# RmSchaffert/ACCV-Lab

Hardware: AMD Instinct MI355X
Metric: heatmap frames/sec (1920x1080 fp32, ragged N_obj in [1,128], fused clear+draw) (higher is better)
Workload: dtype f32

## Files before the change

accv-lab_amd/accvlab/_amd_native/__init__.py:

```python
from __future__ import annotations

import ctypes
import os

_HERE = os.path.dirname(os.path.abspath(__file__))
NO_HOST_FASTPATH = os.environ.get("ACCV_NO_HOST_FASTPATH", "") not in ("", "0")
LIB_PATH = os.environ.get("ACCV_HIP_LIB") or os.path.join(_HERE, "libaccv_hip.so")

OK = 0
HM_CLEAR = 1
HM_COUNTS_I64 = 2
HM_SMALL_RADII = 4
HM_WRITE_THROUGH = 8
HM_GROUP_BOXES_GIVEN = 16
HM_TILE_ROWS_16 = 32
HM_TILE_ROWS_8 = 64
HM_CALLER_SCALE_ORDER = 256
HM_PLAIN_STORES = 128
HM_POINT_COUNTS_I64 = 512
MP_IDX_I64 = 1
MP_COUNTS_I64 = 2
MP_LABELS_I64 = 4
FL_AVG_NUM_POS = 0
FL_AVG_VALUE = 1
FL_AVG_DEVICE = 2
LSA_MAXIMIZE = 1
LSA_THREADS_64 = 2
LSA_THREADS_1024 = 4
MC_ONE_MINUS_PROB = 0
MC_NEG_PROB = 1
MC_FOCAL = 2
MC_LABELS_I64 = 1
MC_CXCYWH = 2
CR_MAX_MAPS = 8
CR_MAX_CHANNELS = 64
CR_COUNTS_I64 = 1
CR_INDEX_FORM = 2
CR_WEIGHTS_PER_CHANNEL = 4
CR_L1 = 0
CR_SMOOTH_L1 = 2
MF_IDX_I64 = 1
MF_LABELS_I64 = 2
MB_IDX_I64 = 1
MB_CXCYWH = 2
MB_IOU_NONE = 0
MB_IOU = 1
MB_GIOU = 2
MB_MAX_D = 16
PM_IDX_I64 = 1
PM_REVERSIBLE = 2
PM_LABELS_I64 = 4
PM_CLOSED_I32 = 8
PM_CLOSED_I64 = 16
PM_MIN_P = 2
PM_MAX_P = 128
CT_MAX_TASKS = 8
CT_MAX_CLASSES = 64
CT_NO_TASK = 255
CT_LABELS_I64 = 1
CT_COUNTS_I64 = 2
CD_MAX_TASKS = 8
CD_MAX_MAPS = 8
CD_MAX_CLASSES = 64
CD_MAX_K = 1024
RN_MAX_TASKS = 8
RN_MAX_N = 1024
RN_MIN_D = 7
RN_MAX_D = 16

_vp = ctypes.c_void_p
_i = ctypes.c_int
_f = ctypes.c_float
_u = ctypes.c_uint
_sz = ctypes.c_size_t
_i64 = ctypes.c_int64
_ll = ctypes.c_longlong
_u64 = ctypes.c_uint64

SIGNATURES = {
    "accv_last_error": (ctypes.c_char_p, []),
    "accv_version": (_i, []),
    "accv_draw_heatmap_last_dispatch": (ctypes.c_char_p, []),
    "accv_draw_heatmap_time_next_launch": (_i, [_vp, _vp]),
    "accv_draw_heatmap_flat_workspace_bytes": (_sz, [_i, _i]),
    "accv_draw_heatmap_flat_f32": (_i, [_vp, _i, _i, _i, _vp, _vp, _vp, _i, _f, _f, _u, _vp, _sz, _vp]),
    "accv_draw_heatmap_batched_f32": (_i, [_vp, _i, _i, _i, _i, _vp, _vp, _vp, _vp, _i, _f, _f, _u, _vp]),
    "accv_fill_f32": (_i, [_vp, _sz, _f, _vp]),
    "accv_draw_heatmap_multiscale_f32": (_i, [_vp, _vp, _vp, _vp, _i, _i, _vp, _vp, _vp, _i, _f, _f, _u, _vp]),
    "accv_draw_heatmap_multiscale_sample_f32": (_i, [_vp, _vp, _vp, _vp, _i, _i, _vp, _vp, _vp, _i, _f, _f, _u,
                                                      _vp, _i, _i, _vp, _i, _vp, _vp, _vp]),
    "accv_draw_points_workspace_bytes": (_sz, [_i, _i]),
    "accv_draw_points_multiscale_f32": (_i, [_vp, _vp, _vp, _vp, _i, _i, _vp, _vp, _i, _i, _f, _f, _u, _vp, _sz, _vp]),
    "accv_draw_polylines_fused_applicable": (_i, [_vp, _vp, _i, _i, _i, _i, _i]),
    "accv_draw_polylines_multiscale_f32": (_i, [_vp, _vp, _vp, _vp, _i, _i, _vp, _i, _i, _vp, _vp, _i, _i, _f, _f, _u, _vp]),
    "accv_heatmap_targets_from_boxes_f32": (_i, [_vp, _vp, _ll, _f, _vp, _vp, _vp]),
    "accv_heatmap_targets_from_points_f32": (_i, [_vp, _ll, _f, _i, _vp, _vp, _vp]),
    "accv_ragged_gather": (_i, [_vp, _vp, _vp, _vp, _ll, _ll, _ll, _ll, _ll, _i, _i, _vp, _vp]),
    "accv_ragged_gather_fill": (_i, [_vp, _vp, _vp, _vp, _ll, _ll, _ll, _ll, _ll, _u64, _i, _i, _i, _vp, _vp]),
    "accv_ragged_scatter": (_i, [_vp, _vp, _vp, _vp, _ll, _ll, _ll, _ll, _ll, _i, _i, _vp, _vp]),
    "accv_ragged_map_pairs": (_i, [_vp, _vp, _vp, _vp, _vp, _ll, _ll, _ll, _ll, _ll, _ll, _i, _i, _vp, _vp]),
    "accv_ragged_insert_const": (_i, [_vp, _vp, _vp, _ll, _ll, _ll, _ll, _ll, _u64, _i, _i, _i, _vp, _vp]),
    "accv_ragged_pad_fill": (_i, [_vp, _vp, _ll, _ll, _ll, _u64, _i, _i, _vp]),
# ... 290 lines not shown
```

accv-lab_amd/accvlab/draw_heatmap/ops.py:

```python
from __future__ import annotations

import ctypes
from typing import Optional

import torch

from .. import _amd_native as _nat

try:
    from . import _dh_host as _dh
except ImportError:
    _dh = None
_native_bound = False


def _native():
    global _native_bound
    if _dh is None or _nat.NO_HOST_FASTPATH:
        return None
    if not _native_bound:
        h = _nat.ctypes_lib()
        addr = lambda name: ctypes.cast(getattr(h, name), ctypes.c_void_p).value
        _dh.bind_native(addr("accv_draw_heatmap_batched_f32"), addr("accv_last_error"))
        _native_bound = True
    return _dh


_FORCED_FLAGS = 0


def _hint_flags(clear: bool, small_radii: bool, write_through: bool, tile_rows) -> int:
    if tile_rows not in (None, 8, 16):
        raise RuntimeError("tile_rows must be None, 8 or 16")
    return (_nat.HM_CLEAR if clear else 0) | (_nat.HM_SMALL_RADII if small_radii else 0) | \
        (0 if write_through is None else _nat.HM_WRITE_THROUGH if write_through else _nat.HM_PLAIN_STORES) | \
        (_nat.HM_TILE_ROWS_16 if tile_rows == 16 else _nat.HM_TILE_ROWS_8 if tile_rows == 8 else 0) | _FORCED_FLAGS


def _one_launch_maps(maps, batch: int, device):
    k = len(maps)
    if not 1 <= k <= 4:
        return None
    ptrs, hs, ws = [], [], []
    for hm in maps:
        if not (isinstance(hm, torch.Tensor) and hm.is_cuda and hm.dtype == torch.float32 and hm.is_contiguous() and
                hm.device == device):
            return None
        shape = hm.shape
        if len(shape) != 3 or shape[0] != batch:
            return None
        ptr = hm.data_ptr()
        if shape[2] % 4 or ptr % 16 or shape[1] * shape[2] * 4 >= (1 << 31):
            return None
        ptrs.append(ptr)
        hs.append(shape[1])
        ws.append(shape[2])
    return (ctypes.c_void_p * k)(*ptrs), (ctypes.c_int * k)(*hs), (ctypes.c_int * k)(*ws)


def _check_maps(maps, batch: int, device, owner: str) -> None:
    for hm in maps:
        _check_input(hm, "heatmap")
        _check_dtype(hm, torch.float32, "heatmap")
        if not (hm.dim() == 3 and hm.size(0) == batch):
            raise RuntimeError("every heatmap must be of shape [batch_size, height, width]")
        if not (hm.device == device):
            raise RuntimeError(f"every heatmap must be on the {owner}' device ({device})")


def _require(cond: bool, msg: str) -> None:
    if not cond:
        raise RuntimeError(msg)


def _check_input(t: torch.Tensor, name: str) -> None:
    if not (isinstance(t, torch.Tensor)):
        raise RuntimeError(f"{name} must be a torch.Tensor")
    if not (t.is_cuda):
        raise RuntimeError(f"{name} must be a CUDA tensor")
    if not (t.is_contiguous()):
        raise RuntimeError(f"{name} must be contiguous")


def _check_dtype(t: torch.Tensor, dtype: torch.dtype, name: str) -> None:
    if not (t.dtype == dtype):
        raise RuntimeError(f"{name}: expected scalar type {dtype} but found {t.dtype}")


def _same_device(ref: torch.Tensor, *others) -> None:
    for name, t in others:
        if not (t.device == ref.device):
            raise RuntimeError(f"{name} must be on the same device as the heatmap ({ref.device})")


_FLAT_DIRECT_MAX_OBJECTS = 2048
_FLAT_DIRECT_MAX_ROUNDS = 200_000
_constants: dict = {}


def _flat_direct(planes: int, height: int, width: int, n: int) -> bool:
    if not (0 < n <= _FLAT_DIRECT_MAX_OBJECTS and 0 < planes <= 65535 and height > 0 and width > 0):
        return False
    tiles = planes * ((width + 127) // 128) * ((height + 15) // 16)
    return tiles * ((n + 63) // 64) <= _FLAT_DIRECT_MAX_ROUNDS


def _device_constant(key, make) -> torch.Tensor:
    t = _constants.get(key)
    if t is None:
        t = make()
        if torch.cuda.is_current_stream_capturing():
            return t
        torch.cuda.current_stream(t.device).synchronize()
        if len(_constants) > 256:
            _constants.clear()
        _constants[key] = t
    return t


def draw_heatmap(
    heatmaps: torch.Tensor,
    centers: torch.Tensor,
    radii: torch.Tensor,
    heatmap_idxes: torch.Tensor,
    diameter_to_sigma_factor: float = 6.0,
    k_scale: float = 1.0,
    *,
    clear: bool = False,
    small_radii: bool = False,
    write_through: Optional[bool] = None,
    tile_rows: Optional[int] = None,
) -> None:
    _check_input(heatmaps, "heatmap")
    _check_input(centers, "centers")
    _check_input(radii, "radii")
    _check_input(heatmap_idxes, "heatmap_idxes")
    if not (centers.size(0) == radii.size(0)):
        raise RuntimeError("centers and radii must have the same size at dim0")
    if not (centers.size(0) == heatmap_idxes.size(0)):
        raise RuntimeError("centers and heatmap_idxes must have the same size at dim0")
    if not (heatmaps.dim() == 3):
        raise RuntimeError("heatmap must be of shape [num_heatmaps, height, width]")
    if not (centers.dim() == 2 and centers.size(1) == 2):
        raise RuntimeError("centers must be of shape [num_targets, 2]")
    if not (radii.dim() == 1 and heatmap_idxes.dim() == 1):
        raise RuntimeError("radii and heatmap_idxes must be of shape [num_targets]")
    _check_dtype(heatmaps, torch.float32, "heatmap")
    _check_dtype(centers, torch.int32, "centers")
    _check_dtype(radii, torch.int32, "radii")
    _check_dtype(heatmap_idxes, torch.int32, "heatmap_idxes")
    _same_device(heatmaps, ("centers", centers), ("radii", radii), ("heatmap_idxes", heatmap_idxes))

    lib = _nat.lib()
    planes, height, width = heatmaps.shape
    n = centers.size(0)
    if _flat_direct(planes, height, width, n):
        with _nat.device_guard(heatmaps.device):
            dev = heatmaps.device
            count = _device_constant(("count", n, dev), lambda: torch.full((1,), n, dtype=torch.int32, device=dev))
            status = lib.accv_draw_heatmap_batched_f32(
                heatmaps.data_ptr(), 1, planes, height, width, centers.data_ptr(), radii.data_ptr(), count.data_ptr(),
                heatmap_idxes.data_ptr(), n, float(diameter_to_sigma_factor), float(k_scale),
                _hint_flags(clear, small_radii, write_through, tile_rows), _nat.stream_ptr(heatmaps.device))
        _nat.check(status, "draw_heatmap")
        return
    with _nat.device_guard(heatmaps.device):
        ws_bytes = lib.accv_draw_heatmap_flat_workspace_bytes(planes, n)
        ws = torch.empty(ws_bytes, dtype=torch.uint8, device=heatmaps.device)
        status = lib.accv_draw_heatmap_flat_f32(
            heatmaps.data_ptr(), planes, height, width, centers.data_ptr(), radii.data_ptr(),
            heatmap_idxes.data_ptr(), n, float(diameter_to_sigma_factor), float(k_scale),
            _hint_flags(clear, small_radii, write_through, tile_rows), ws.data_ptr(), ws_bytes,
            _nat.stream_ptr(heatmaps.device))
    _nat.check(status, "draw_heatmap")


def draw_heatmap_batched(
    heatmap: torch.Tensor,
    centers,
    radii,
    diameter_to_sigma_factor: float = 6.0,
    k_scale: float = 1.0,
    labels=None,
    *,
    clear: bool = False,
    small_radii: bool = False,
    write_through: Optional[bool] = None,
    tile_rows: Optional[int] = None,
) -> None:
    centers_t = centers.tensor
    radii_t = radii.tensor
    assert centers_t.shape[0] == radii_t.shape[0], "centers and radii must have the same size batch size"
    assert centers_t.shape[1] == radii_t.shape[1], "centers and radii must have the same maximum number of objects"
    counts = centers.sample_sizes
    labels_t: Optional[torch.Tensor] = None
    if labels is not None:
        labels_t = labels.tensor
        assert centers_t.shape[0] == labels_t.shape[0], "centers and labels must have the same size batch size"
        assert centers_t.shape[1] == labels_t.shape[1], \
            "centers and labels must have the same maximum number of objects"

    native = _native()
    if native is not None and isinstance(heatmap, torch.Tensor) and isinstance(counts, torch.Tensor) and \
            native.draw_batched(heatmap, centers_t, radii_t, counts, labels_t, float(diameter_to_sigma_factor), float(k_scale),
                                _hint_flags(clear, small_radii, write_through, tile_rows)):
        return

    if counts.dtype not in (torch.int32, torch.int64):
        counts = counts.to(torch.int64)

    _check_input(heatmap, "heatmap")
    _check_input(centers_t, "centers")
    _check_input(radii_t, "radii")
    _check_input(counts, "nums_targets")
    batch = heatmap.size(0)
    n_max = radii_t.size(1) if radii_t.dim() >= 2 else -1
    _require(batch == radii_t.size(0) and batch == centers_t.size(0) and batch == counts.size(0),
             "batch_size (dim 0) need to be the same for all inputs")
    if not (centers_t.dim() == 3 and centers_t.size(2) == 2):
        raise RuntimeError("centers must be of shape [batch_size, num_targets, 2]")
    if not (radii_t.dim() == 2):
        raise RuntimeError("radii must be of shape [batch_size, num_targets]")
    if not (n_max == centers_t.size(1)):
        raise RuntimeError("maximum number of targets (dim 1) need to be the same centers and radii")
    if not (counts.dim() == 1):
        raise RuntimeError("nums_targets must be of shape [batch_size]")
    _check_dtype(heatmap, torch.float32, "heatmap")
    _check_dtype(centers_t, torch.int32, "centers")
    _check_dtype(radii_t, torch.int32, "radii")
    others = [("centers", centers_t), ("radii", radii_t), ("nums_targets", counts)]
    if labels_t is None:
        if not (heatmap.dim() == 3):
            raise RuntimeError("heatmap must be of shape [batch_size, height, width]")
        num_classes, (height, width) = 0, heatmap.shape[1:]
        labels_ptr = None
    else:
        _check_input(labels_t, "labels")
        if not (heatmap.dim() == 4):
            raise RuntimeError("heatmap must be of shape [batch_size, max_num_classes, height, width]")
        if not (labels_t.dim() == 2):
            raise RuntimeError("labels must be of shape [batch_size, radii.size(1)]")
        _require(labels_t.size(0) == batch and labels_t.size(1) == n_max,
                 "labels shape must be [batch_size, radii.size(1)]")
        _check_dtype(labels_t, torch.int32, "labels")
        num_classes, height, width = heatmap.shape[1:]
        if not (num_classes > 0 or heatmap.numel() == 0):
            raise RuntimeError("class-wise heatmap needs at least one class plane")
        labels_ptr = labels_t.data_ptr()
        others.append(("labels", labels_t))
    _same_device(heatmap, *others)
    if labels_t is not None and num_classes == 0:
        return

    flags = _hint_flags(clear, small_radii, write_through, tile_rows) | \
        (_nat.HM_COUNTS_I64 if counts.dtype == torch.int64 else 0)
    with _nat.device_guard(heatmap.device):
        status = _nat.lib().accv_draw_heatmap_batched_f32(
            heatmap.data_ptr(), batch, num_classes, height, width, centers_t.data_ptr(), radii_t.data_ptr(),
            counts.data_ptr(), labels_ptr, n_max, float(diameter_to_sigma_factor), float(k_scale), flags,
            _nat.stream_ptr(heatmap.device))
    _nat.check(status, "draw_heatmap_batched")


def get_centers_and_radii(centers, bboxes, out_size_factor: float):
    ragged = hasattr(centers, "tensor") and hasattr(centers, "create_with_sample_sizes_like_self")
    c_t = centers.tensor if ragged else centers
    b_t = bboxes.tensor if hasattr(bboxes, "tensor") else bboxes
    _require(c_t.shape[-1] == 2 and b_t.shape[-1] == 4 and c_t.shape[:-1] == b_t.shape[:-1],
             "centers must be [..., 2] and bboxes [..., 4] with equal leading dimensions")
    if c_t.is_cuda:
        if not (b_t.device == c_t.device):
            raise RuntimeError("centers and bboxes must be on the same device")
        c32 = c_t.to(torch.float32).contiguous()
        b32 = b_t.to(torch.float32).contiguous()
        out_c = torch.empty(c32.shape, dtype=torch.int32, device=c32.device)
        out_r = torch.empty(c32.shape[:-1], dtype=torch.int32, device=c32.device)
        with _nat.device_guard(c32.device):
            _nat.check(_nat.lib().accv_heatmap_targets_from_boxes_f32(
                c32.data_ptr(), b32.data_ptr(), out_r.numel(), float(out_size_factor), out_c.data_ptr(),
                out_r.data_ptr(), _nat.stream_ptr(c32.device)), "get_centers_and_radii")
    else:
        d = torch.cat([c_t - b_t[..., :2], b_t[..., 2:] - c_t], dim=-1)
        out_r = torch.ceil(torch.min(d, dim=-1)[0] / out_size_factor).to(torch.int32).clamp_(min=1)
        out_c = (c_t / out_size_factor).to(torch.int32)
    if ragged:
        nu = centers.non_uniform_dim
        return centers.create_with_sample_sizes_like_self(out_c, nu), centers.create_with_sample_sizes_like_self(out_r, nu)
    return out_c, out_r


def draw_heatmap_multiscale(heatmaps, centers, bboxes, out_size_factors, diameter_to_sigma_factor: float = 6.0,
                            k_scale: float = 1.0, *, clear: bool = False) -> None:
    heatmaps = list(heatmaps)
    strides = [float(f) for f in out_size_factors]
    if not (len(heatmaps) == len(strides) and len(heatmaps) >= 1):
        raise RuntimeError("heatmaps and out_size_factors must have the same, non-zero length")
    objects = _box_objects(centers, bboxes)
    batch, dev = objects[0].size(0), objects[0].device
    geometry = _one_launch_maps(heatmaps, batch, dev)
    if geometry is None:
        _check_maps(heatmaps, batch, dev, "centers")
        for hm, f in zip(heatmaps, strides):
            ci, ri = get_centers_and_radii(centers, bboxes, f)
            draw_heatmap_batched(hm, ci, ri, diameter_to_sigma_factor, k_scale, clear=clear)
        return
    _launch_box_maps(geometry, strides, objects, diameter_to_sigma_factor, k_scale, clear)


def _box_objects(centers, bboxes):
    c_t = centers.tensor
    b_t = bboxes.tensor if hasattr(bboxes, "tensor") else bboxes
    counts = centers.sample_sizes
    if counts.dtype not in (torch.int32, torch.int64):
        counts = counts.to(torch.int64)
    _check_input(c_t, "centers")
    _check_input(b_t, "bboxes")
    _check_input(counts, "nums_targets")
    if not (c_t.dim() == 3 and c_t.size(2) == 2):
        raise RuntimeError("centers must be of shape [batch_size, num_targets, 2]")
    if not (b_t.dim() == 3 and b_t.size(2) == 4 and b_t.shape[:2] == c_t.shape[:2]):
        raise RuntimeError("bboxes must be of shape [batch_size, num_targets, 4]")
    _check_dtype(c_t, torch.float32, "centers")
    _check_dtype(b_t, torch.float32, "bboxes")
    if not (counts.dim() == 1 and counts.size(0) == c_t.size(0)):
        raise RuntimeError("nums_targets must be of shape [batch_size]")
    _same_device(c_t, ("bboxes", b_t), ("nums_targets", counts))
    return c_t, b_t, counts


def _launch_box_maps(geometry, strides, objects, diameter_to_sigma_factor, k_scale, clear, job=None) -> None:
    ptrs, hs, ws = geometry
    c_t, b_t, counts = objects
    batch, n_max = c_t.shape[:2]
    n = len(strides)
    st = (ctypes.c_float * n)(*strides)
    flags = (_nat.HM_CLEAR if clear else 0) | (_nat.HM_COUNTS_I64 if counts.dtype == torch.int64 else 0) | _FORCED_FLAGS
    dev = c_t.device
# ... 13 lines not shown
```

accv-lab_amd/csrc/draw_heatmap.hip:

```cpp
#include <hip/hip_runtime.h>
#include <hip/hip_ext.h>

#include <algorithm>
#include <atomic>
#include <climits>
#include <cstdint>
#include <cstring>
#include <type_traits>

#include "accv_common.h"
#include "splat_common.h"
#include "splat_stamps.h"
#include "splat_tile.h"
#include "splat_small.h"
#include "splat_lanes.h"
#include "heatmap_prep.h"

namespace {

void note_dispatch(const char* kernel, int px, int r, bool clear, int sm, const dim3& grid, const dim3& block)
{
    snprintf(accv::dispatch_buffer(), 256, "%s<PX=%d,R=%d,CLEAR=%d,SM=%d> grid(%u,%u,%u) block(%u)", kernel, px, r, clear ? 1 : 0,
             sm, grid.x, grid.y, grid.z, block.x);
}

struct LaunchEvents {
    hipEvent_t start = nullptr, stop = nullptr;
};
LaunchEvents& launch_events()
{
    static thread_local LaunchEvents ev;
    return ev;
}
LaunchEvents take_launch_events()
{
    const LaunchEvents ev = launch_events();
    launch_events() = LaunchEvents{};
    return ev;
}
template <class K>
inline void launch_maybe_timed(K kernel, const dim3& grid, const dim3& block, hipStream_t stream, const LaunchEvents& ev,
                               const SplatParams& p)
{
    if (ev.start || ev.stop)
        hipExtLaunchKernelGGL(kernel, grid, block, 0, stream, ev.start, ev.stop, 0, p);
    else
        hipLaunchKernelGGL(kernel, grid, block, 0, stream, p);
}
template <class F>
void with_variant(bool clear, bool write_through, F&& f)
{
    using Plain = std::integral_constant<int, kStorePlain>;
    using WriteThrough = std::integral_constant<int, kStoreWriteThrough>;
    if (clear && write_through)
        f(std::true_type{}, WriteThrough{});
    else if (clear)
        f(std::true_type{}, Plain{});
    else if (write_through)
        f(std::false_type{}, WriteThrough{});
    else
        f(std::false_type{}, Plain{});
}

int launch_splat_small(SplatParams p, long long planes, bool clear, bool write_through, hipStream_t stream, const LaunchEvents& ev)
{
    p.tiles_x = (p.W + 127) / 128;
    p.tiles_y = (p.H + 15) / 16;
    p.n_tiles = planes * p.tiles_x * p.tiles_y;
    if (p.n_tiles == 0) return ACCV_OK;
    dim3 grid;
    p.grid3d = (planes <= 65535 && p.tiles_y <= 65535) ? 1 : 0;
    if (p.grid3d) {
        grid = dim3((unsigned)p.tiles_x, (unsigned)p.tiles_y, (unsigned)planes);
    } else {
        if (p.n_tiles > INT_MAX) return accv::fail(ACCV_EINVAL, "draw_heatmap: %lld tiles exceed the grid limit", p.n_tiles);
        grid = dim3((unsigned)p.n_tiles);
    }
    with_variant(clear, write_through, [&](auto CL, auto SM) {
        launch_maybe_timed(splat_small_kernel<CL, SM>, grid, dim3(64), stream, ev, p);
    });
    note_dispatch("splat_small_kernel", 4, 8, clear, write_through ? kStoreWriteThrough : kStorePlain, grid, dim3(64));
    return accv::check_launch("draw_heatmap small-splat kernel");
}

template <int PX, int R>
int launch_splat(SplatParams p, long long planes, bool clear, int sm, hipStream_t stream, const LaunchEvents& ev)
{
    p.tiles_x = (p.W + 32 * PX - 1) / (32 * PX);
    p.tiles_y = (p.H + 2 * R - 1) / (2 * R);
    p.n_tiles = planes * p.tiles_x * p.tiles_y;
    if (p.n_tiles == 0) return ACCV_OK;
    const int groups_x = (p.tiles_x + kWavesPerGroup - 1) / kWavesPerGroup;
    dim3 grid, block(kWavesPerGroup * 64);
    p.grid3d = (planes <= 65535 && p.tiles_y <= 65535) ? 1 : 0;
    if (p.grid3d) {
        grid = dim3((unsigned)groups_x, (unsigned)p.tiles_y, (unsigned)planes);
    } else {
        const long long groups = (p.n_tiles + kWavesPerGroup - 1) / kWavesPerGroup;
        if (groups > INT_MAX) return accv::fail(ACCV_EINVAL, "draw_heatmap: %lld tiles exceed the grid limit", p.n_tiles);
        grid = dim3((unsigned)groups);
    }
    attach_splat_stamps(p);
    if (PX == 1 || (sm == kStoreAdaptive && clear)) sm = kStorePlain;
    if (sm == kStoreAdaptive) {
        if constexpr (PX == 4) launch_maybe_timed(splat_kernel<PX, R, false, kStoreAdaptive>, grid, block, stream, ev, p);
    } else {
        with_variant(clear, sm == kStoreWriteThrough, [&](auto CL, auto SM) {
            if constexpr (PX == 4 || SM == kStorePlain) launch_maybe_timed(splat_kernel<PX, R, CL, SM>, grid, block, stream, ev, p);
        });
    }
    note_dispatch("splat_kernel", PX, R, clear, sm, grid, block);
    return accv::check_launch("draw_heatmap splat kernel");
}

long long compute_units()
{
    static std::atomic<int> cached[64];
    int dev = 0;
    if (hipGetDevice(&dev) != hipSuccess || dev < 0 || dev >= 64) return 0;
    int v = cached[dev].load(std::memory_order_relaxed);
    if (v == 0) {
        int n = 0;
        if (hipDeviceGetAttribute(&n, hipDeviceAttributeMultiprocessorCount, dev) != hipSuccess || n <= 0) return 0;
        cached[dev].store(n, std::memory_order_relaxed);
        v = n;
    }
    return v;
}

int dispatch_splat(SplatParams p, long long planes, bool clear, unsigned flags, hipStream_t stream, const LaunchEvents& ev)
{
    const bool small_hint = (flags & ACCV_HM_SMALL_RADII) != 0;
    const bool vec4 = (p.W % 4 == 0) && ((reinterpret_cast<uintptr_t>(p.hm) & 15u) == 0);
    const bool plane_fits_rsrc = (size_t)p.H * p.W * sizeof(float) < ((size_t)1 << 31);
    int nt;
    if (flags & ACCV_HM_WRITE_THROUGH)
        nt = kStoreWriteThrough;
    else if (flags & ACCV_HM_PLAIN_STORES)
        nt = kStorePlain;
    else
        nt = clear ? kStorePlain : kStoreAdaptive;
    if (nt != kStorePlain && !plane_fits_rsrc) nt = kStorePlain;
    p.dense_area = 0.75f * (float)p.H * (float)p.W;
    int rows = (flags & ACCV_HM_TILE_ROWS_16) ? 16 : 8;
    if (!(flags & (ACCV_HM_TILE_ROWS_8 | ACCV_HM_TILE_ROWS_16)) && clear && vec4 && !small_hint) {
        const long long cus = compute_units();
        const long long tx = (p.W + 127) / 128;
        const long long tiles8 = planes * tx * ((p.H + 15) / 16), tiles16 = planes * tx * ((p.H + 31) / 32);
        if (cus > 0 && tiles8 > 24 * cus && tiles16 <= 16 * cus) rows = 16;
    }
    if (!p.labels) p.labels = p.radii;
    if (!vec4) return launch_splat<1, 8>(p, planes, clear, kStorePlain, stream, ev);
    if (small_hint) return launch_splat_small(p, planes, clear, nt == kStoreWriteThrough, stream, ev);
    if (rows == 16) return launch_splat<4, 16>(p, planes, clear, nt, stream, ev);
    return launch_splat<4, 8>(p, planes, clear, nt, stream, ev);
}

int check_common(int h, int w, const char* who)
{
    if (h < 0 || w < 0) return accv::fail(ACCV_EINVAL, "%s: negative heatmap extent %dx%d", who, h, w);
    if (h > (1 << 29) || w > (1 << 29))
        return accv::fail(ACCV_EINVAL, "%s: heatmap extent %dx%d exceeds 2^29 per dimension", who, h, w);
    return ACCV_OK;
}

inline void coarse_scales_first(MultiParams& mp)
{
    std::stable_sort(mp.scale, mp.scale + mp.n_scales,
                     [](const SplatParams& a, const SplatParams& b) { return a.n_tiles < b.n_tiles; });
    long long tiles = 0;
    for (int i = 0; i < mp.n_scales; ++i) {
        mp.tile_begin[i] = tiles;
        tiles += mp.scale[i].n_tiles;
    }
    mp.tile_begin[mp.n_scales] = tiles;
}
inline void seal_tile_prefix(MultiParams& mp)
{
    for (int i = mp.n_scales + 1; i <= kMaxScales; ++i) mp.tile_begin[i] = mp.tile_begin[mp.n_scales];
}

inline int multiscale_store_mode(unsigned flags) { return (flags & ACCV_HM_WRITE_THROUGH) ? kStoreWriteThrough : kStorePlain; }

constexpr const char* kPerScaleNote = " (use the per-scale calls otherwise)";
long long setup_scales(MultiParams& mp, const SplatParams& proto, float* const* heatmaps, const int* heights, const int* widths,
                       const float* strides, int num_scales, int batch, int tile_h, unsigned flags, const char* who,
                       const char* map_note)
{
    long long tiles = 0;
    int used = 0;
    for (int i = 0; i < num_scales; ++i) {
        if (int rc = check_common(heights[i], widths[i], who)) return rc;
        if (!(strides[i] > 0.0f)) return accv::fail(ACCV_EINVAL, "%s: stride %d is not positive", who, i);
        if (heights[i] == 0 || widths[i] == 0) continue;
        if (!heatmaps[i]) return accv::fail(ACCV_EINVAL, "%s: heatmap %d is null", who, i);
        if (widths[i] % 4 != 0 || (reinterpret_cast<uintptr_t>(heatmaps[i]) & 15u) ||
            (size_t)heights[i] * widths[i] * sizeof(float) >= ((size_t)1 << 31))
            return accv::fail(ACCV_EINVAL, "%s: map %d needs a width that is a multiple of 4, a 16-byte aligned base and planes "
                                           "below 2 GiB%s", who, i, map_note);
        SplatParams& p = mp.scale[used];
        p = proto;
        p.hm = heatmaps[i];
        p.H = heights[i];
        p.W = widths[i];
        p.stride = strides[i];
        p.tiles_x = (p.W + 127) / 128;
        p.tiles_y = (p.H + tile_h - 1) / tile_h;
        p.n_tiles = (long long)batch * p.tiles_x * p.tiles_y;
        p.grid3d = 0;
        mp.tile_begin[used] = tiles;
        tiles += p.n_tiles;
        ++used;
    }
    mp.n_scales = used;
    mp.tile_begin[used] = tiles;
    if (!(flags & ACCV_HM_CALLER_SCALE_ORDER)) coarse_scales_first(mp);
    seal_tile_prefix(mp);
    return tiles;
}

int check_scale_arrays(const char* who, float* const* heatmaps, const int* heights, const int* widths, const float* strides,
                       int num_scales)
{
    if (num_scales < 1 || num_scales > kMaxScales)
        return accv::fail(ACCV_EINVAL, "%s: 1..%d scales supported, got %d", who, kMaxScales, num_scales);
    if (!heatmaps || !heights || !widths || !strides) return accv::fail(ACCV_EINVAL, "%s: null array", who);
    return ACCV_OK;
}
int check_scale_counts(const char* who, int batch, int per_sample, const char* what)
{
    if (batch < 0 || per_sample < 0) return accv::fail(ACCV_EINVAL, "%s: negative count", who);
    if (per_sample > (1 << 30)) return accv::fail(ACCV_EINVAL, "%s: more than 2^30 %s per sample", who, what);
    return ACCV_OK;
}
SplatParams multiscale_proto(const void* counts, int n_max, float diameter_to_sigma_factor, float k_scale, unsigned flags)
{
// ... 424 lines not shown
```

accv-lab_amd/csrc/splat_common.h:

```cpp
#pragma once
#include <hip/hip_runtime.h>

#include <cstdint>

#include "accv_common.h"

namespace {

constexpr int kWavesPerGroup = 1;
constexpr int kBoxTileR = 8;
constexpr int kCand = 64;
constexpr float kLog2e = 1.4426950408889634f;

constexpr int kSrcObjects = 0;
constexpr int kSrcFloatBoxes = 1;
constexpr int kSrcPoints = 2;
constexpr int kStorePlain = 0;
constexpr int kStoreWriteThrough = 4;
constexpr int kStoreAdaptive = 5;

struct SplatParams {
    float* hm;
    const int32_t* centers;
    const int32_t* radii;
    const int32_t* labels;
    const void* counts;
    const int32_t* plane_off;
    int H, W;
    int n_max;
    int n_classes;
    int tiles_x, tiles_y;
    long long n_tiles;
    float factor, k;
    int counts_i64;
    int grid3d;
    float dense_area;
    const float* centers_f;
    const float* boxes_f;
    float stride;
    int radius, n_groups;
#ifdef ACCV_SPLAT_STAMPS
    unsigned long long* stamps;
    long long stamp_records;
#endif
};

constexpr int kMaxScales = 4;
struct MultiParams {
    SplatParams scale[kMaxScales];
    long long tile_begin[kMaxScales + 1];
    int n_scales;
};

struct __attribute__((aligned(16))) Hit {
    int x, y;
    float c2;
    unsigned box;
};

template <int PX>
struct Vec;
typedef float vfloat4 __attribute__((ext_vector_type(4)));
template <>
struct Vec<4> {
    using type = vfloat4;
};
template <>
struct Vec<1> {
    using type = float;
};

__device__ __forceinline__ float raw_exp2(float x) { return __builtin_amdgcn_exp2f(x); }

__device__ __forceinline__ float max_skip_nan(float acc, float v)
{
    float r;
    asm("v_max_f32 %0, %1, %2" : "=v"(r) : "v"(acc), "v"(v));
    return r;
}

struct TileCtx {
    int tx0, ty0, tx1, ty1;
    long long plane;
    const int2* centers2;
    const int32_t* radii;
    const int32_t* labels;
    const float2* centers_f;
    const float4* boxes_f;
    float4 box0;
    float stride;
    int radius;
    int n, cls;
};

template <bool SCALAR_COUNT = false>
__device__ __forceinline__ void plane_objects(const SplatParams& p, TileCtx& t);

template <int TW, int TH, int WPG, bool SCALAR_COUNT = false>
__device__ __forceinline__ bool locate_tile(const SplatParams& p, int wave, TileCtx& t, long long linear_group)
{
    int tx, ty;
    if (p.grid3d) {
        tx = blockIdx.x * WPG + wave;
        ty = blockIdx.y;
        t.plane = blockIdx.z;
        if (tx >= p.tiles_x) return false;
    } else {
        const long long tile = linear_group * WPG + wave;
        if (tile >= p.n_tiles) return false;
        if (p.n_tiles <= 0x7fffffffll) {
            const unsigned t32 = (unsigned)tile, t2 = t32 / (unsigned)p.tiles_x;
            tx = (int)(t32 - t2 * (unsigned)p.tiles_x);
            const unsigned pl = t2 / (unsigned)p.tiles_y;
            ty = (int)(t2 - pl * (unsigned)p.tiles_y);
            t.plane = pl;
        } else {
            tx = (int)(tile % p.tiles_x);
            const long long t2 = tile / p.tiles_x;
            ty = (int)(t2 % p.tiles_y);
            t.plane = t2 / p.tiles_y;
        }
    }
    t.tx0 = tx * TW;
// ... 40 lines not shown
    t.boxes_f = reinterpret_cast<const float4*>(p.boxes_f) + (p.n_groups > 0 ? (t.plane * p.n_groups) : obj_base);
    t.stride = p.stride;
    t.radius = p.radius;
}

struct Cand {
    int x, y, r, label;
};
template <int SRC = kSrcObjects>
__device__ __forceinline__ Cand cull_load(const TileCtx& t, int base, int lane)
{
    const int cc = min(base + lane, t.n - 1);
    if constexpr (SRC == kSrcFloatBoxes) {
        const float2 c = t.centers_f[cc];
        const float4 b = t.boxes_f[cc];
        const float m = fminf(fminf(c.x - b.x, c.y - b.y), fminf(b.z - c.x, b.w - c.y));
        const bool pow2 = (__float_as_uint(t.stride) & 0x007fffffu) == 0u && t.stride > 1.0e-30f && t.stride < 1.0e30f;
        if (pow2) {
            const float inv = 1.0f / t.stride;
            int r = (int)ceilf(m * inv);
            if (r < 1) r = 1;
            return Cand{(int)(c.x * inv), (int)(c.y * inv), r, 0};
        }
        int r = (int)ceilf(__fdiv_rn(m, t.stride));
        if (r < 1) r = 1;
        return Cand{(int)__fdiv_rn(c.x, t.stride), (int)__fdiv_rn(c.y, t.stride), r, 0};
    } else if constexpr (SRC == kSrcPoints) {
        const float2 c = t.centers_f[cc];
        const bool bad = (c.x != c.x) || (c.y != c.y);
        if (bad) return Cand{0, 0, -1, 0};
        return Cand{(int)__fdiv_rn(c.x, t.stride), (int)__fdiv_rn(c.y, t.stride), t.radius, 0};
    } else {
        const int2 cxy = t.centers2[cc];
        return Cand{cxy.x, cxy.y, t.radii[cc], t.labels[cc]};
    }
}
__device__ __forceinline__ unsigned long long cull_test(const TileCtx& t, int base, int lane, const Cand& c)
{
    constexpr int kClampXY = 1 << 29, kClampR = 1 << 30;
    const int xc = min(max(c.x, -kClampXY), kClampXY), yc = min(max(c.y, -kClampXY), kClampXY);
    const int rc = min(c.r, kClampR);
    const bool hit = (base + lane < t.n) && (t.cls < 0 || c.label == t.cls) && c.r >= 0 && xc - rc < t.tx1 &&
                     xc + rc >= t.tx0 && yc - rc < t.ty1 && yc + rc >= t.ty0;
    return __ballot(hit);
}
template <int SRC = kSrcObjects>
__device__ __forceinline__ unsigned long long cull_round(const TileCtx& t, int base, int lane, int& x, int& y, int& r)
{
    const Cand c = cull_load<SRC>(t, base, lane);
    x = c.x;
    y = c.y;
    r = c.r;
    return cull_test(t, base, lane, c);
}

__device__ __forceinline__ float hit_exponent_scale(const SplatParams& p, int r)
{
    const float sigma = (float)(2 * r + 1) / p.factor;
    return kLog2e / (2.0f * sigma * sigma);
}
__device__ __forceinline__ Hit make_hit(const SplatParams& p, const TileCtx& t, int x, int y, int r, float c2);
__device__ __forceinline__ Hit make_hit(const SplatParams& p, const TileCtx& t, int x, int y, int r)
{
    return make_hit(p, t, x, y, r, hit_exponent_scale(p, r));
}
__device__ __forceinline__ Hit make_hit(const SplatParams& p, const TileCtx& t, int x, int y, int r, float c2)
{
    const long long x0 = (long long)x - min(x, r), x1 = (long long)x + min((long long)p.W - x, (long long)r + 1);
    const long long y0 = (long long)y - min(y, r), y1 = (long long)y + min((long long)p.H - y, (long long)r + 1);
    const long long xlo = max(x0, (long long)t.tx0) - t.tx0, xhi = min(x1, (long long)t.tx1) - t.tx0;
    const long long ylo = max(y0, (long long)t.ty0) - t.ty0, yhi = min(y1, (long long)t.ty1) - t.ty0;
    unsigned box = 0;
    if (xhi > xlo && yhi > ylo) box = (unsigned)xlo | ((unsigned)xhi << 8) | ((unsigned)ylo << 16) | ((unsigned)yhi << 24);
    return Hit{x, y, c2, box};
}

__device__ __forceinline__ float max3_skip_nan(float acc, float a, float b)
{
    float r;
    asm("v_max3_f32 %0, %1, %2, %3" : "=v"(r) : "v"(acc), "v"(a), "v"(b));
    return r;
}

__device__ __forceinline__ int scale_of_group(const MultiParams& mp, long long group, long long& first)
{
    int s = 0;
    first = 0;
#pragma unroll
    for (int i = 1; i < kMaxScales; ++i) {
        const long long begin = mp.tile_begin[i];
        if (group >= begin) {
            s = i;
            first = begin;
        }
    }
    return s;
}
template <typename T>
__device__ __forceinline__ void pin_scalar(T& v)
{
    asm volatile("" : "+s"(v));
}
__device__ __forceinline__ SplatParams preload_params(const SplatParams& src)
{
    SplatParams p = src;
    asm volatile("" ::"s"(p.hm), "s"(p.counts), "s"(p.centers_f), "s"(p.boxes_f));
    pin_scalar(p.H);
    pin_scalar(p.W);
    pin_scalar(p.n_max);
    pin_scalar(p.n_classes);
    pin_scalar(p.tiles_x);
    pin_scalar(p.tiles_y);
    pin_scalar(p.n_tiles);
    pin_scalar(p.factor);
    pin_scalar(p.k);
    pin_scalar(p.counts_i64);
    pin_scalar(p.grid3d);
    pin_scalar(p.dense_area);
    pin_scalar(p.stride);
    pin_scalar(p.radius);
    pin_scalar(p.n_groups);
    return p;
}

constexpr int kDppQuad0 = 0x00, kDppQuad1 = 0x55, kDppQuad2 = 0xAA, kDppQuad3 = 0xFF;
constexpr int kDppRowShr = 0x110;
constexpr int kDppWaveShl1 = 0x130, kDppWaveShr1 = 0x138;
template <int CTRL>
__device__ __forceinline__ float dpp_f(float old, float src)
{
    return __int_as_float(__builtin_amdgcn_update_dpp(__float_as_int(old), __float_as_int(src), CTRL, 0xf, 0xf, false));
}
template <int CTRL>
__device__ __forceinline__ int dpp_i(int old, int src)
{
    return __builtin_amdgcn_update_dpp(old, src, CTRL, 0xf, 0xf, false);
}

}
```

accv-lab_amd/csrc/splat_tile.h:

```cpp
#pragma once

namespace {

template <int PX, int R, bool CLEAR, int SM, int WPG, int SRC>
__device__ __forceinline__ void splat_body(const SplatParams& p, long long linear_group)
{
    constexpr int kWavesPerGroup = WPG;
    constexpr int TW = 32 * PX;
    constexpr int TH = 2 * R;
    static_assert(R % 4 == 0, "row registers are fetched four at a time");

    __shared__ Hit s_hit[kWavesPerGroup][kCand];
    __shared__ __attribute__((aligned(16))) float s_ey[kWavesPerGroup][kCand][TH];

    constexpr bool kSharedColumns = CLEAR && SRC == kSrcObjects && PX == 4;
    PhaseStamps<kSplatStampsBuilt && CLEAR && SRC == kSrcObjects && PX == 4> stamps;
    stamps.start();
    const int lane = threadIdx.x & 63;
    const int wave = __builtin_amdgcn_readfirstlane(threadIdx.x >> 6);
    TileCtx t;
    if (!locate_tile<TW, TH, kWavesPerGroup>(p, wave, t, linear_group)) return;
    const int tx0 = t.tx0, ty0 = t.ty0, n = t.n;
    const long long plane = t.plane;

    const int sub = lane >> 5;
    const int col0 = tx0 + (lane & 31) * PX;

    float acc[R][PX];
    const float init = CLEAR ? 0.0f : __builtin_nanf("");
#pragma unroll
    for (int i = 0; i < R; ++i)
#pragma unroll
        for (int c = 0; c < PX; ++c) acc[i][c] = init;

    int total_hits = 0;
    float cover = 0.0f;

    for (int base = 0; base < n; base += kCand) {
        int x, y, r;
        const unsigned long long m = cull_round<SRC>(t, base, lane, x, y, r);
        if constexpr (SM == kStoreAdaptive) {
            const float dia = (float)(2 * min(max(r, 0), 1 << 20) + 1);
            cover += (base + lane < n) ? dia * dia : 0.0f;
        }
        const bool hit = (m >> lane) & 1ull;
        const int nh = __popcll(m);
        stamps.cull();
        if (nh == 0) continue;
        if constexpr (!CLEAR) {
            if (total_hits == 0 && col0 < p.W) {
                const float* plane_rd = p.hm + (size_t)plane * (size_t)p.H * (size_t)p.W;
#pragma unroll
                for (int i = 0; i < R; ++i) {
                    const int row = ty0 + sub * R + i;
                    if (row < p.H) {
                        if constexpr (PX == 4) {
                            const vfloat4 o = *reinterpret_cast<const vfloat4*>(plane_rd + (size_t)row * p.W + col0);
                            acc[i][0] = o.x;
                            acc[i][1] = o.y;
                            acc[i][2] = o.z;
                            acc[i][3] = o.w;
                        } else {
                            acc[i][0] = plane_rd[(size_t)row * p.W + col0];
                        }
                    }
                }
            }
        }
        if (hit) s_hit[wave][__popcll(m & ((1ull << lane) - 1ull))] = make_hit(p, t, x, y, r);
        __builtin_amdgcn_fence(__ATOMIC_RELEASE, "wavefront");
        __builtin_amdgcn_fence(__ATOMIC_ACQUIRE, "wavefront");

        for (int t = lane; t < nh * TH; t += 64) {
            const int h = t / TH, rr = t % TH;
            const Hit hy = s_hit[wave][h];
            const float d = (float)(ty0 + rr - hy.y);
            const float v = p.k * raw_exp2(-(d * d) * hy.c2);
            const unsigned ylo = (hy.box >> 16) & 255u, yhi = hy.box >> 24;
            s_ey[wave][h][rr] = ((unsigned)rr >= ylo && (unsigned)rr < yhi) ? v : __builtin_nanf("");
        }
        __builtin_amdgcn_fence(__ATOMIC_RELEASE, "wavefront");
        __builtin_amdgcn_fence(__ATOMIC_ACQUIRE, "wavefront");
        stamps.table();

        const unsigned colr0 = (unsigned)(lane & 31) * PX;
        auto column_factors = [&](const Hit& hx, float (&ex)[PX]) {
            const unsigned xlo = hx.box & 255u, xhi = (hx.box >> 8) & 255u;
#pragma unroll
            for (int c = 0; c < PX; ++c) {
                const float d = (float)(col0 + c - hx.x);
                const float e = raw_exp2(-(d * d) * hx.c2);
                ex[c] = (colr0 + c >= xlo && colr0 + c < xhi) ? e : __builtin_nanf("");
            }
        };
        [[maybe_unused]] auto column_factors_shared = [&](const Hit& hx, float (&ex)[PX]) {
            if constexpr (PX == 4) {
                const unsigned xlo = hx.box & 255u, xhi = (hx.box >> 8) & 255u;
                unsigned f[2];
#pragma unroll
                for (int j = 0; j < 2; ++j) {
                    const int c = 2 * sub + j;
                    const float d = (float)(col0 + c - hx.x);
                    const float e = raw_exp2(-(d * d) * hx.c2);
                    f[j] = __float_as_uint((colr0 + c >= xlo && colr0 + c < xhi) ? e : __builtin_nanf(""));
                }
#pragma unroll
                for (int j = 0; j < 2; ++j) {
                    const auto sw = __builtin_amdgcn_permlane32_swap(f[j], f[j], false, false);
                    ex[j] = __uint_as_float(sw[0]);
                    ex[2 + j] = __uint_as_float(sw[1]);
                }
            }
        };
        int h = 0;
        for (; CLEAR && h + 1 < nh; h += 2) {
            float exa[PX], exb[PX];
            if constexpr (kSharedColumns) {
                column_factors_shared(s_hit[wave][h], exa);
                column_factors_shared(s_hit[wave][h + 1], exb);
            } else {
                column_factors(s_hit[wave][h], exa);
                column_factors(s_hit[wave][h + 1], exb);
            }
#pragma unroll
            for (int q = 0; q < R / 4; ++q) {
                const float4 a4 = *reinterpret_cast<const float4*>(&s_ey[wave][h][sub * R + 4 * q]);
                const float4 b4 = *reinterpret_cast<const float4*>(&s_ey[wave][h + 1][sub * R + 4 * q]);
                const float eya[4] = {a4.x, a4.y, a4.z, a4.w}, eyb[4] = {b4.x, b4.y, b4.z, b4.w};
#pragma unroll
                for (int i = 0; i < 4; ++i)
#pragma unroll
                    for (int c = 0; c < PX; ++c)
                        acc[4 * q + i][c] = max3_skip_nan(acc[4 * q + i][c], exa[c] * eya[i], exb[c] * eyb[i]);
            }
        }
        for (; h < nh; ++h) {
            float ex[PX];
            if constexpr (kSharedColumns)
                column_factors_shared(s_hit[wave][h], ex);
            else
                column_factors(s_hit[wave][h], ex);
#pragma unroll
            for (int q = 0; q < R / 4; ++q) {
                const float4 e4 = *reinterpret_cast<const float4*>(&s_ey[wave][h][sub * R + 4 * q]);
                const float ey[4] = {e4.x, e4.y, e4.z, e4.w};
#pragma unroll
                for (int i = 0; i < 4; ++i)
#pragma unroll
                    for (int c = 0; c < PX; ++c) acc[4 * q + i][c] = max_skip_nan(acc[4 * q + i][c], ex[c] * ey[i]);
            }
        }
        total_hits += nh;
        stamps.accumulate();
        __builtin_amdgcn_fence(__ATOMIC_RELEASE, "wavefront");
        __builtin_amdgcn_fence(__ATOMIC_ACQUIRE, "wavefront");
    }

    if (!CLEAR && total_hits == 0) return;
    if (col0 >= p.W) return;

    using V = typename Vec<PX>::type;
    float* plane_ptr = p.hm + (size_t)plane * (size_t)p.H * (size_t)p.W;
    bool write_through = SM == kStoreWriteThrough;
    if constexpr (SM == kStoreAdaptive && PX == 4) {
#pragma unroll
        for (int d = 32; d >= 1; d >>= 1) cover += __shfl_xor(cover, d);
        write_through = cover >= p.dense_area;
    }
// ... 40 lines not shown
```

include/accv_hip.h:

```cpp
#ifndef ACCV_HIP_H
#define ACCV_HIP_H

#include <stddef.h>
#include <stdint.h>

#ifdef __cplusplus
extern "C" {
#endif

#define ACCV_OK 0
#define ACCV_EINVAL (-1)
#define ACCV_ELAUNCH (-2)
#define ACCV_EWORKSPACE (-3)
#define ACCV_ERUNTIME (-4)

#define ACCV_HM_CLEAR 1u
#define ACCV_HM_COUNTS_I64 2u
#define ACCV_HM_SMALL_RADII 4u
#define ACCV_HM_WRITE_THROUGH 8u
#define ACCV_HM_GROUP_BOXES_GIVEN 16u

#define ACCV_HM_PLAIN_STORES 128u
#define ACCV_HM_TILE_ROWS_16 32u
#define ACCV_HM_TILE_ROWS_8 64u
#define ACCV_HM_CALLER_SCALE_ORDER 256u

const char* accv_last_error(void);
int accv_version(void);
const char* accv_draw_heatmap_last_dispatch(void);


int accv_draw_heatmap_time_next_launch(void* start_event, void* stop_event);

size_t accv_draw_heatmap_flat_workspace_bytes(int num_planes, int num_objects);
int accv_draw_heatmap_flat_f32(float* heatmaps, int num_planes, int height, int width, const int32_t* centers,
                               const int32_t* radii, const int32_t* heatmap_idxes, int num_objects,
                               float diameter_to_sigma_factor, float k_scale, unsigned flags, void* workspace,
                               size_t workspace_bytes, void* stream);

int accv_draw_heatmap_batched_f32(float* heatmap, int batch, int num_classes, int height, int width,
                                  const int32_t* centers, const int32_t* radii, const void* counts,
                                  const int32_t* labels, int max_num_targets, float diameter_to_sigma_factor,
                                  float k_scale, unsigned flags, void* stream);

int accv_draw_heatmap_multiscale_f32(float* const* heatmaps, const int* heights, const int* widths, const float* strides,
                                     int num_scales, int batch, const float* centers_xy, const float* boxes_xyxy,
                                     const void* counts, int max_num_targets, float diameter_to_sigma_factor,
                                     float k_scale, unsigned flags, void* stream);

int accv_draw_heatmap_multiscale_sample_f32(float* const* heatmaps, const int* heights, const int* widths, const float* strides,
                                            int num_scales, int batch, const float* centers_xy, const float* boxes_xyxy,
                                            const void* counts, int max_num_targets, float diameter_to_sigma_factor,
                                            float k_scale, unsigned flags, const float* polylines_xy, int num_polylines,
                                            int points, const void* point_counts, int num_samples, float* samples,
                                            float* group_boxes, void* stream);

size_t accv_draw_points_workspace_bytes(int batch, int num_points);
int accv_draw_points_multiscale_f32(float* const* heatmaps, const int* heights, const int* widths, const float* strides,
                                    int num_scales, int batch, const float* points_xy, const void* counts, int num_points,
                                    int radius, float diameter_to_sigma_factor, float k_scale, unsigned flags,
                                    void* workspace, size_t workspace_bytes, void* stream);

#define ACCV_HM_POINT_COUNTS_I64 512u
int accv_draw_polylines_fused_applicable(const int* heights, const int* widths, int num_scales, int batch, int lanes,
                                         int points, int num_samples);
int accv_draw_polylines_multiscale_f32(float* const* heatmaps, const int* heights, const int* widths, const float* strides,
                                       int num_scales, int batch, const float* polylines_xy, int lanes, int points,
                                       const void* point_counts, const void* lane_counts, int num_samples, int radius,
                                       float diameter_to_sigma_factor, float k_scale, unsigned flags, void* stream);

int accv_heatmap_targets_from_boxes_f32(const float* centers_xy, const float* boxes_xyxy, long long num_objects,
                                        float stride, int32_t* out_centers, int32_t* out_radii, void* stream);

int accv_heatmap_targets_from_points_f32(const float* points_xy, long long num_points, float stride, int radius,
                                         int32_t* out_centers, int32_t* out_radii, void* stream);


int accv_ragged_gather(const void* src, void* dst, const void* indices, const void* counts, long long batch,
                       long long w_src, long long w_idx, long long idx_stride, long long row_bytes, int idx_i64,
                       int counts_i64, int* err_counter, void* stream);

int accv_ragged_gather_fill(const void* src, void* dst, const void* indices, const void* counts, long long batch,
                            long long w_src, long long w_idx, long long idx_stride, long long row_bytes,
                            uint64_t fill_bits, int elem_size, int idx_i64, int counts_i64, int* err_counter,
                            void* stream);

int accv_ragged_scatter(const void* src, void* dst, const void* indices, const void* counts, long long batch,
                        long long w_idx, long long idx_stride, long long w_dst, long long row_bytes, int idx_i64,
                        int counts_i64, int* err_counter, void* stream);

int accv_ragged_map_pairs(const void* src, void* dst, const void* src_indices, const void* dst_indices,
                          const void* counts, long long batch, long long w_src, long long w_idx, long long idx_stride,
                          long long w_dst, long long row_bytes, int idx_i64, int counts_i64, int* err_counter,
                          void* stream);

int accv_ragged_insert_const(void* dst, const void* indices, const void* counts, long long batch, long long w_idx,
                             long long idx_stride, long long w_dst, long long row_bytes, uint64_t elem_bits,
                             int elem_size, int idx_i64, int counts_i64, int* err_counter, void* stream);

int accv_ragged_pad_fill(void* data, const void* counts, long long batch, long long width, long long row_bytes,
                         uint64_t elem_bits, int elem_size, int counts_i64, void* stream);

int accv_ragged_accumulate(const void* src, void* dst, const void* src_indices_or_null, const void* dst_indices,
                           const void* counts, long long batch, long long w_src, long long w_idx, long long idx_stride,
                           long long w_dst, long long row_elems, int acc_dtype, int idx_i64, int counts_i64,
                           int* err_counter, void* stream);

int accv_ragged_mask_to_indices(const void* mask_u8, const void* valid_counts_or_null, int valid_i64, long long batch,
// ... 369 lines not shown
```

Baseline: 716,800.

## Prune Gaussian hits dominated by another hit within a tile before splatting

Adds a per-tile pass in the splat kernel that checks pairs of hits (8x8 per ballot round) and drops any hit whose Gaussian is provably below another's over the whole tile intersection, with numeric safety margins. Surviving hits are compacted in LDS before the row/column factor evaluation, so dense tiles evaluate fewer Gaussians per pixel. It runs only when a tile has at least four hits and the scale factors are in a safe range, and a new KEEP_DOMINATED flag disables it. The cost is extra pairwise ALU work and ballots per tile, plus a small risk of floating-point differences against the max-reduction reference.

```diff
diff --git a/accv-lab_amd/accvlab/_amd_native/__init__.py b/accv-lab_amd/accvlab/_amd_native/__init__.py
--- a/accv-lab_amd/accvlab/_amd_native/__init__.py
+++ b/accv-lab_amd/accvlab/_amd_native/__init__.py
@@ -18,6 +18,7 @@
 HM_CALLER_SCALE_ORDER = 256
 HM_PLAIN_STORES = 128
 HM_POINT_COUNTS_I64 = 512
+HM_KEEP_DOMINATED = 1024
 MP_IDX_I64 = 1
 MP_COUNTS_I64 = 2
 MP_LABELS_I64 = 4
diff --git a/accv-lab_amd/accvlab/draw_heatmap/ops.py b/accv-lab_amd/accvlab/draw_heatmap/ops.py
--- a/accv-lab_amd/accvlab/draw_heatmap/ops.py
+++ b/accv-lab_amd/accvlab/draw_heatmap/ops.py
@@ -29,12 +29,13 @@
 _FORCED_FLAGS = 0
 
 
-def _hint_flags(clear: bool, small_radii: bool, write_through: bool, tile_rows) -> int:
+def _hint_flags(clear: bool, small_radii: bool, write_through: bool, tile_rows, keep_dominated: bool = False) -> int:
     if tile_rows not in (None, 8, 16):
         raise RuntimeError("tile_rows must be None, 8 or 16")
     return (_nat.HM_CLEAR if clear else 0) | (_nat.HM_SMALL_RADII if small_radii else 0) | \
         (0 if write_through is None else _nat.HM_WRITE_THROUGH if write_through else _nat.HM_PLAIN_STORES) | \
-        (_nat.HM_TILE_ROWS_16 if tile_rows == 16 else _nat.HM_TILE_ROWS_8 if tile_rows == 8 else 0) | _FORCED_FLAGS
+        (_nat.HM_TILE_ROWS_16 if tile_rows == 16 else _nat.HM_TILE_ROWS_8 if tile_rows == 8 else 0) | \
+        (_nat.HM_KEEP_DOMINATED if keep_dominated else 0) | _FORCED_FLAGS
 
 
 def _one_launch_maps(maps, batch: int, device):
@@ -130,6 +131,7 @@
     small_radii: bool = False,
     write_through: Optional[bool] = None,
     tile_rows: Optional[int] = None,
+    keep_dominated: bool = False,
 ) -> None:
     _check_input(heatmaps, "heatmap")
     _check_input(centers, "centers")
@@ -161,7 +163,7 @@
             status = lib.accv_draw_heatmap_batched_f32(
                 heatmaps.data_ptr(), 1, planes, height, width, centers.data_ptr(), radii.data_ptr(), count.data_ptr(),
                 heatmap_idxes.data_ptr(), n, float(diameter_to_sigma_factor), float(k_scale),
-                _hint_flags(clear, small_radii, write_through, tile_rows), _nat.stream_ptr(heatmaps.device))
+                _hint_flags(clear, small_radii, write_through, tile_rows, keep_dominated), _nat.stream_ptr(heatmaps.device))
         _nat.check(status, "draw_heatmap")
         return
     with _nat.device_guard(heatmaps.device):
@@ -170,7 +172,7 @@
         status = lib.accv_draw_heatmap_flat_f32(
             heatmaps.data_ptr(), planes, height, width, centers.data_ptr(), radii.data_ptr(),
             heatmap_idxes.data_ptr(), n, float(diameter_to_sigma_factor), float(k_scale),
-            _hint_flags(clear, small_radii, write_through, tile_rows), ws.data_ptr(), ws_bytes,
+            _hint_flags(clear, small_radii, write_through, tile_rows, keep_dominated), ws.data_ptr(), ws_bytes,
             _nat.stream_ptr(heatmaps.device))
     _nat.check(status, "draw_heatmap")
 
@@ -187,6 +189,7 @@
     small_radii: bool = False,
     write_through: Optional[bool] = None,
     tile_rows: Optional[int] = None,
+    keep_dominated: bool = False,
 ) -> None:
     centers_t = centers.tensor
     radii_t = radii.tensor
@@ -203,7 +206,7 @@
     native = _native()
     if native is not None and isinstance(heatmap, torch.Tensor) and isinstance(counts, torch.Tensor) and \
             native.draw_batched(heatmap, centers_t, radii_t, counts, labels_t, float(diameter_to_sigma_factor), float(k_scale),
-                                _hint_flags(clear, small_radii, write_through, tile_rows)):
+                                _hint_flags(clear, small_radii, write_through, tile_rows, keep_dominated)):
         return
 
     if counts.dtype not in (torch.int32, torch.int64):
@@ -252,7 +255,7 @@
     if labels_t is not None and num_classes == 0:
         return
 
-    flags = _hint_flags(clear, small_radii, write_through, tile_rows) | \
+    flags = _hint_flags(clear, small_radii, write_through, tile_rows, keep_dominated) | \
         (_nat.HM_COUNTS_I64 if counts.dtype == torch.int64 else 0)
     with _nat.device_guard(heatmap.device):
         status = _nat.lib().accv_draw_heatmap_batched_f32(
diff --git a/accv-lab_amd/csrc/draw_heatmap.hip b/accv-lab_amd/csrc/draw_heatmap.hip
--- a/accv-lab_amd/csrc/draw_heatmap.hip
+++ b/accv-lab_amd/csrc/draw_heatmap.hip
@@ -3,6 +3,7 @@
 
 #include <algorithm>
 #include <atomic>
+#include <cfloat>
 #include <climits>
 #include <cstdint>
 #include <cstring>
@@ -142,6 +143,8 @@
         nt = clear ? kStorePlain : kStoreAdaptive;
     if (nt != kStorePlain && !plane_fits_rsrc) nt = kStorePlain;
     p.dense_area = 0.75f * (float)p.H * (float)p.W;
+    const bool may_prune = !(flags & ACCV_HM_KEEP_DOMINATED) && p.k >= 0x1p-32f && p.k <= 0x1p32f && p.factor > 0.0f &&
+                           p.factor <= FLT_MAX;
     int rows = (flags & ACCV_HM_TILE_ROWS_16) ? 16 : 8;
     if (!(flags & (ACCV_HM_TILE_ROWS_8 | ACCV_HM_TILE_ROWS_16)) && clear && vec4 && !small_hint) {
         const long long cus = compute_units();
@@ -152,6 +155,7 @@
     if (!p.labels) p.labels = p.radii;
     if (!vec4) return launch_splat<1, 8>(p, planes, clear, kStorePlain, stream, ev);
     if (small_hint) return launch_splat_small(p, planes, clear, nt == kStoreWriteThrough, stream, ev);
+    p.prune = may_prune ? kPruneMinHits : 0;
     if (rows == 16) return launch_splat<4, 16>(p, planes, clear, nt, stream, ev);
     return launch_splat<4, 8>(p, planes, clear, nt, stream, ev);
 }
diff --git a/accv-lab_amd/csrc/splat_common.h b/accv-lab_amd/csrc/splat_common.h
--- a/accv-lab_amd/csrc/splat_common.h
+++ b/accv-lab_amd/csrc/splat_common.h
@@ -39,6 +39,7 @@
     const float* boxes_f;
     float stride;
     int radius, n_groups;
+    int prune;
 #ifdef ACCV_SPLAT_STAMPS
     unsigned long long* stamps;
     long long stamp_records;
@@ -245,6 +246,89 @@
     return r;
 }
 
+constexpr int kPruneDominators = 8;
+#ifndef ACCV_PRUNE_MIN_HITS
+#define ACCV_PRUNE_MIN_HITS 4
+#endif
+constexpr int kPruneMinHits = ACCV_PRUNE_MIN_HITS;
+static_assert(kPruneMinHits >= 2, "a pair needs two hits");
+constexpr float kPruneMargin = 0x1.4p-10f;
+constexpr float kPruneMaxExponent = 40.0f;
+struct AxisBound {
+    float q;
+    float eh;
+    float s;
+    float m;
+};
+__device__ __forceinline__ AxisBound dominance_axis(int lo, int hi, int xg, int xh, float cg, float ch, float a, float rca, float cs)
+{
+    const float dgl = (float)(int)((unsigned)lo - (unsigned)xg), dgh = (float)(int)((unsigned)hi - (unsigned)xg);
+    const float dhl = (float)(int)((unsigned)lo - (unsigned)xh), dhh = (float)(int)((unsigned)hi - (unsigned)xh);
+    AxisBound b;
+    b.m = fmaxf(fmaxf(fabsf(dgl), fabsf(dgh)), fmaxf(fabsf(dhl), fabsf(dhh)));
+    const float egl = (dgl * dgl) * cg, egh = (dgh * dgh) * cg, ehl = (dhl * dhl) * ch, ehh = (dhh * dhh) * ch;
+    b.q = fminf(egl - ehl, egh - ehh);
+    b.eh = fmaxf(ehl, ehh);
+    b.s = (egl + egh) + (ehl + ehh);
+    const float sl = fmaf(cg, dgl, -(ch * dhl)), sh = fmaf(cg, dgh, -(ch * dhh));
+    const float tol = cs * b.m;
+    const bool vertex = a > 0.0f && !(sl >= tol) && !(sh <= -tol);
+    const float dc = dgl - dhl;
+    const float v = -(rca * (ch * (dc * dc)));
+    if (vertex) {
+        b.q = fminf(b.q, v);
+        b.s += fabsf(v);
+    }
+    return b;
+}
+__device__ __forceinline__ bool hit_dominated(const Hit& g, const Hit& h, int tx0, int ty0)
+{
+    const unsigned gxl = g.box & 255u, gxh = (g.box >> 8) & 255u, gyl = (g.box >> 16) & 255u, gyh = g.box >> 24;
+    const unsigned hxl = h.box & 255u, hxh = (h.box >> 8) & 255u, hyl = (h.box >> 16) & 255u, hyh = h.box >> 24;
+    const bool contained = hxl <= gxl && hxh >= gxh && hyl <= gyl && hyh >= gyh;
+    const float cg = g.c2, ch = h.c2, a = cg - ch;
+    const float rca = cg * __builtin_amdgcn_rcpf(a), cs = (cg + ch) * 0x1p-20f;
+    float q = 0.0f, s = 0.0f, eh = 0.0f, m = 0.0f;
+#pragma nounroll
+    for (int ax = 0; ax < 2; ++ax) {
+        const unsigned gb = g.box >> (16 * ax);
+        const int org = ax ? ty0 : tx0;
+        const AxisBound b = dominance_axis(org + (int)(gb & 255u), org + (int)((gb >> 8) & 255u) - 1, ax ? g.y : g.x,
+                                           ax ? h.y : h.x, cg, ch, a, rca, cs);
+        q += b.q;
+        s += b.s;
+        eh = fmaxf(eh, b.eh);
+        m = fmaxf(m, b.m);
+    }
+    return contained && m <= 0x1p23f && eh <= kPruneMaxExponent &&
+           q - s * 0x1p-20f >= kPruneMargin;
+}
+__device__ __forceinline__ int prune_dominated(Hit* hits, int nh, int lane, int tx0, int ty0)
+{
+    static_assert(kPruneDominators == 8, "a byte of the ballot per hit");
+    const int hi = lane & 7, gsub = lane >> 3;
+    bool dom = false;
+    for (int g0 = 0; g0 < nh; g0 += 8) {
+        const int gi = g0 + gsub;
+        const Hit h = hits[min(hi, nh - 1)], g = hits[min(gi, nh - 1)];
+        const bool d = gi < nh && hi < nh && hi != gi && hit_dominated(g, h, tx0, ty0);
+        const unsigned long long b = __ballot(d);
+        if (gsub == (g0 >> 3)) dom = ((b >> (8 * hi)) & 0xffull) != 0ull;
+    }
+    const bool keep = lane < nh && !dom;
+    const unsigned long long km = __ballot(keep);
+    const int kept = __popcll(km);
+    if (kept != nh) {
+        typedef unsigned raw4 __attribute__((ext_vector_type(4)));
+        raw4* slots = reinterpret_cast<raw4*>(hits);
+        const raw4 mine = slots[min(lane, nh - 1)];
+        if (keep) slots[__popcll(km & ((1ull << lane) - 1ull))] = mine;
+        __builtin_amdgcn_fence(__ATOMIC_RELEASE, "wavefront");
+        __builtin_amdgcn_fence(__ATOMIC_ACQUIRE, "wavefront");
+    }
+    return kept;
+}
+
 __device__ __forceinline__ int scale_of_group(const MultiParams& mp, long long group, long long& first)
 {
     int s = 0;
diff --git a/accv-lab_amd/csrc/splat_tile.h b/accv-lab_amd/csrc/splat_tile.h
--- a/accv-lab_amd/csrc/splat_tile.h
+++ b/accv-lab_amd/csrc/splat_tile.h
@@ -44,7 +44,7 @@
             cover += (base + lane < n) ? dia * dia : 0.0f;
         }
         const bool hit = (m >> lane) & 1ull;
-        const int nh = __popcll(m);
+        int nh = __popcll(m);
         stamps.cull();
         if (nh == 0) continue;
         if constexpr (!CLEAR) {
@@ -71,7 +71,14 @@
         __builtin_amdgcn_fence(__ATOMIC_RELEASE, "wavefront");
         __builtin_amdgcn_fence(__ATOMIC_ACQUIRE, "wavefront");
 
-        for (int t = lane; t < nh * TH; t += 64) {
+        if constexpr (kSharedColumns) {
+            if (p.prune && nh >= p.prune) nh = prune_dominated(s_hit[wave], nh, lane, tx0, ty0);
+        }
+        int ln = lane;
+        if constexpr (kSharedColumns) asm volatile("" : "+v"(ln));
+        const int sub = ln >> 5, col0 = tx0 + (ln & 31) * PX;
+
+        for (int t = ln; t < nh * TH; t += 64) {
             const int h = t / TH, rr = t % TH;
             const Hit hy = s_hit[wave][h];
             const float d = (float)(ty0 + rr - hy.y);
@@ -83,7 +90,7 @@
         __builtin_amdgcn_fence(__ATOMIC_ACQUIRE, "wavefront");
         stamps.table();
 
-        const unsigned colr0 = (unsigned)(lane & 31) * PX;
+        const unsigned colr0 = (unsigned)(ln & 31) * PX;
         auto column_factors = [&](const Hit& hx, float (&ex)[PX]) {
             const unsigned xlo = hx.box & 255u, xhi = (hx.box >> 8) & 255u;
 #pragma unroll
diff --git a/include/accv_hip.h b/include/accv_hip.h
--- a/include/accv_hip.h
+++ b/include/accv_hip.h
@@ -24,6 +24,7 @@
 #define ACCV_HM_TILE_ROWS_16 32u
 #define ACCV_HM_TILE_ROWS_8 64u
 #define ACCV_HM_CALLER_SCALE_ORDER 256u
+#define ACCV_HM_KEEP_DOMINATED 1024u
 
 const char* accv_last_error(void);
 int accv_version(void);
```

Result: no change. 721,700, median of 6 (+0.7%).
